# SensorsINI/v2e

Hardware: NVIDIA H100
Metric: Mevents/s (higher is better)
Workload: dtype fp16 tensor-core convs (fp32 accumulate) + f64 pixel state

## Files before the change

### include/v2e_b200.h

```cpp
#ifndef V2E_B200_H
#define V2E_B200_H

#include <stdint.h>

#ifdef __cplusplus
extern "C" {
#endif

typedef enum V2eStatus {
    V2E_OK = 0,
    V2E_E_INVALID = -1,
    V2E_E_CUDA = -2,
    V2E_E_CAPACITY = -3,
    V2E_E_ITER_CAP = -4,
    V2E_E_STATE = -5,
    V2E_E_UNSUPPORTED = -6,
    V2E_E_FALLBACK = -7
} V2eStatus;

typedef enum V2eFrameDtype { V2E_U8 = 0, V2E_F32 = 1, V2E_F64 = 2 } V2eFrameDtype;

const char *v2e_last_error(void);
int v2e_version(void);
int v2e_abi_info(int *version, int *emu_cfg_size, int *frame_info_size, int *unet_weights_size);
// ... 122 lines not shown
    V2E_CONV_TILE_LEGACY = 0,
    V2E_CONV_TILE_256x128 = 1,
    V2E_CONV_TILE_128x256 = 2
};
int v2e_conv2d_lrelu_sm100_tile(const void *x1_dev, int C1, const void *x2_dev, int C2,
                                const void *wgt_dev, const float *bias_dev, int Cout_pad, int KH, int KW,
                                int N, int H, int W, void *out_dev, int out_cstride, int out_mode,
                                int co_real, float slope, int tile, int multicast, void *stream);
int v2e_conv_pick_tile(int C1, int C2, int Cout_pad, int KH, int KW, int N, int H, int W, int n_sms);

int v2e_conv2d_lrelu_sm100_strip(const void *x1_dev, int C1, const void *x2_dev, int C2,
                                 const void *wgt_row_dev, const float *bias_dev, int Cout_pad, int KH,
                                 int KW, int N, int H, int W, void *out_dev, int out_cstride,
                                 int out_mode, int co_real, float slope, void *stream);
int v2e_conv_strip_pick_kc(int C1, int C2, int Cout_pad, int KH, int KW, int W);

int v2e_conv2d_up2_lrelu_sm100(const void *x_low_dev, int C, const void *wgt_fold_dev, const void *wgt_plain_dev,
                               const float *bias_dev, int Cout_pad, int N, int H_out, int W_out, void *out_dev,
                               int out_cstride, float slope, void *stream);
int v2e_conv_up2_fold_weights(const float *w_host, int cout, int cin, int Cout_pad, int C_pad, void *out_host);
int v2e_conv_up2_supported_c(int C, int Cout_pad, int W_out);

typedef struct V2eUNetWeights {
    const float *w[23];
    const float *b[23];
} V2eUNetWeights;

typedef struct V2eSlomo V2eSlomo;

int v2e_slomo_create(int H, int W, int max_batch, const V2eUNetWeights *flow,
// ... 65 lines not shown
```

### v2e_b200/_lib.py

```python
import ctypes
import os

from . import build as _build

_LIB = None


class V2eEmuCfg(ctypes.Structure):
    _fields_ = [
        ("width", ctypes.c_int32), ("height", ctypes.c_int32),
        ("per_pixel_thres", ctypes.c_int32), ("hdr", ctypes.c_int32),
        ("pos_thres_nominal", ctypes.c_double), ("neg_thres_nominal", ctypes.c_double),
        ("cutoff_hz", ctypes.c_double), ("leak_rate_hz", ctypes.c_double),
        ("leak_jitter_fraction", ctypes.c_double), ("refractory_period_s", ctypes.c_double),
        ("shot_noise_rate_hz", ctypes.c_double), ("shot_inten_factor", ctypes.c_double),
        ("rng_mode", ctypes.c_int32), ("iter_cap", ctypes.c_int32),
        ("seed", ctypes.c_uint64),
        ("csdvs", ctypes.c_int32), ("max_frames_per_step", ctypes.c_int32),
        ("cs_tau_p_s", ctypes.c_double), ("cs_tau_h_s", ctypes.c_double),
        ("scidvs", ctypes.c_int32), ("photoreceptor_noise", ctypes.c_int32),
        ("rng_pixel_offset", ctypes.c_uint32), ("full_frame_px", ctypes.c_uint32),
        ("own_row0", ctypes.c_int32), ("own_rows", ctypes.c_int32),
        ("cs_halo_rows", ctypes.c_int32), ("reserved1", ctypes.c_int32),
    ]
# ... 53 lines not shown
    "v2e_emu_cs_max_dev": (_vp, [_vp]),
    "v2e_emu_cs_advance": (_i, [_vp, _i, _i, _vp]),
    "v2e_emu_cs_update": (_i, [_vp, _vp, _i, _vp, _vp, _vp]),
    "v2e_emu_phase_filter": (_i, [_vp, _d, _d, _u64, _i, _vp]),
    "v2e_emu_read_counts": (_i, [_vp, ctypes.POINTER(ctypes.c_int32), _vp, _i, _vp]),
    "v2e_emu_phase_shot": (_i, [_vp, _vp, _i, _d, _d, _vp, _u64, _vp]),
    "v2e_emu_phase_emit": (_i, [_vp, _d, _d, _vp, _u64, _vp]),
    "v2e_conv2d_lrelu_sm100": (_i, [_vp, _i, _vp, _i, _vp, _vp, _i, _i, _i, _i, _i, _i, _vp, _i, _i, _i,
                                    ctypes.c_float, _vp]),
    "v2e_conv2d_lrelu_sm100_tile": (_i, [_vp, _i, _vp, _i, _vp, _vp, _i, _i, _i, _i, _i, _i, _vp, _i, _i, _i,
                                         ctypes.c_float, _i, _i, _vp]),
    "v2e_conv_pick_tile": (_i, [_i, _i, _i, _i, _i, _i, _i, _i, _i]),
    "v2e_conv2d_lrelu_sm100_strip": (_i, [_vp, _i, _vp, _i, _vp, _vp, _i, _i, _i, _i, _i, _i, _vp, _i, _i, _i,
                                          ctypes.c_float, _vp]),
    "v2e_conv_strip_pick_kc": (_i, [_i, _i, _i, _i, _i, _i]),
    "v2e_conv2d_up2_lrelu_sm100": (_i, [_vp, _i, _vp, _vp, _vp, _i, _i, _i, _i, _vp, _i, ctypes.c_float, _vp]),
    "v2e_conv_up2_fold_weights": (_i, [_vp, _i, _i, _i, _i, _vp]),
    "v2e_conv_up2_supported_c": (_i, [_i, _i, _i]),
    "v2e_slomo_create": (_i, [_i, _i, _i, _vp, _vp, ctypes.POINTER(_vp)]),
    "v2e_slomo_destroy": (_i, [_vp]),
    "v2e_slomo_set_pairs": (_i, [_vp, _vp, _i, _vp]),
    "v2e_slomo_max_flow": (_i, [_vp, ctypes.POINTER(ctypes.c_float), _vp]),
    "v2e_slomo_interp": (_i, [_vp, _d, _vp, _vp, _vp]),
    "v2e_slomo_set_option": (_i, [_vp, _i, _i]),
    "v2e_slomo_check_finite": (_i, [_vp, ctypes.POINTER(_i), _vp]),
    "v2e_slomo_profile": (_i, [_vp, _i]),
    "v2e_slomo_profile_read": (_i, [_vp, ctypes.POINTER(ctypes.c_float), ctypes.POINTER(_i),
                                    ctypes.POINTER(ctypes.c_double), _vp]),
    "v2e_slomo_profile_read_layers": (_i, [_vp, ctypes.POINTER(ctypes.c_float), ctypes.POINTER(_i),
                                           ctypes.POINTER(ctypes.c_double), ctypes.POINTER(ctypes.c_float),
# ... 80 lines not shown
```

### v2e_b200/csrc/conv_tc.cu

```cuda
#include <cuda.h>
#include <cuda_fp16.h>
#include <cuda_runtime.h>
#include <math.h>
#include <stdint.h>
#include <stdio.h>
#include <string.h>
#include <vector>
#include <stdlib.h>

#include "../../include/v2e_b200.h"
#include "common.cuh"
#include "tc_common.cuh"

namespace {

constexpr int kTileH = 8, kTileW = 16, kBM = kTileH * kTileW;
constexpr int kStages = 4;
constexpr int kConvThreads = 288;
constexpr int kProducerWarp = 8;
constexpr int kConsumerWarps = 8;

struct ConvParams {
    int N, H, W;
    int C1, C2;
// ... 255 lines not shown

constexpr int kRowTile = 128;

struct StripParams {
    int N, H, W;
    int C1, C2;
    int KH, KW;
    int KC, BN;
    int tiles_x, seg_h, n_seg, n_items;
    int nslot;
    void *pool_out;
    int pool_cstride;
    int n_split, cout_pad;
    int slab_bytes;
    int w_bytes;
    int out_cstride, out_mode, co_real;
    float slope;
    const float *bias;
    void *out;
};
constexpr int kMaxSlot = 12;
constexpr int kStripThreads = 288;

struct RowRing {
    uint64_t *full, *empty;
    uint32_t nslot, cnt;
    int waited, released;
    __device__ __forceinline__ uint32_t slot(int i) const { return (cnt + (uint32_t)i) % nslot; }
    __device__ __forceinline__ void wait_upto(int n) {
        for (; waited < n; waited++) {
            const uint32_t g = cnt + (uint32_t)waited;
            mbar_wait(&full[g % nslot], (g / nslot) & 1u);
        }
    }
    __device__ __forceinline__ void release_upto(int n, int lane) {
        wait_upto(n);
        __syncwarp();
        for (; released < n; released++)
            if (lane == 0) mbar_arrive(&empty[slot(released)]);
    }
};

template <int KW, int KC, int BN>
__device__ __forceinline__ void strip_pair_mma(float (&acc)[2][BN / 2], const RowRing &rr, int row0, int last, int slabs,
                                               uint64_t dr, uint64_t dw, uint32_t a_off, uint32_t row16, uint32_t slab16) {
    constexpr int KH = KW, taps = KH * KW;
    constexpr uint32_t rowb16 = (KC * 2u) >> 4, tile16 = (BN * KC * 2u) >> 4;
#pragma unroll
    for (int k = 0; k < 2; k++) {
#pragma unroll
        for (int i = 0; i < BN / 2; i++) acc[k][i] = 0.f;
        wgmma_fence_regs(acc[k]);
    }
    wgmma_fence();
#pragma unroll
    for (int rp = 0; rp <= KH; rp++) {
        const uint32_t a_row = rr.slot(row0 + (rp < KH ? rp : last)) * row16 + a_off;
        int sl = 0;
#pragma unroll 1
        do {
            const uint32_t a_lo = a_row + (uint32_t)sl * slab16;
#pragma unroll
            for (int s = 0; s < KW; s++) {
#pragma unroll
                for (int j = 0; j < KC / 16; j++) {
                    const uint64_t ad = desc_add(dr, a_lo + (uint32_t)s * rowb16 + 2u * j);
                    if (rp < KH) wgmma_f16<BN>(acc[0], ad, desc_add(dw, (uint32_t)(sl * taps + rp * KW + s) * tile16 + 2u * j), 1u);
                    if (rp > 0) wgmma_f16<BN>(acc[1], ad, desc_add(dw, (uint32_t)(sl * taps + (rp - 1) * KW + s) * tile16 + 2u * j), 1u);
                }
            }
        } while (++sl < slabs);
    }
    wgmma_commit();
}

template <int KW, int KC, int BN, bool POOL>
__global__ void __launch_bounds__(kStripThreads, 1)
conv_strip_kernel(const __grid_constant__ CUtensorMap tmA, const __grid_constant__ CUtensorMap tmA2,
                  const __grid_constant__ CUtensorMap tmB, const StripParams p) {
    extern __shared__ __align__(1024) uint8_t smem_raw[];
    uint8_t *smem = align1024(smem_raw);
    __shared__ __align__(8) uint64_t full_bar[kMaxSlot], empty_bar[kMaxSlot], w_bar;

    constexpr int KH = KW, ph = KH / 2, pw = KW / 2, taps = KH * KW;
    constexpr int PW = kRowTile + KW - 1;
    constexpr uint32_t tile_bytes = BN * KC * 2;
    const int warp = threadIdx.x >> 5, lane = threadIdx.x & 31;
    const int slabs = (p.C1 + p.C2) / KC;
    const uint32_t row_bytes = (uint32_t)p.slab_bytes * slabs;
    uint8_t *ring = smem + ((p.w_bytes + 1023) & ~1023);
    const int split = (int)blockIdx.x % p.n_split, co_off = split * BN;
    const int item0 = (int)blockIdx.x / p.n_split, item_step = (int)gridDim.x / p.n_split;

    if (threadIdx.x == 0) {
        for (int s = 0; s < p.nslot; s++) { mbar_init(&full_bar[s], 1); mbar_init(&empty_bar[s], kConsumerWarps); }
        mbar_init(&w_bar, 1);
        fence_barrier_init();
    }
    if (warp == kProducerWarp && lane == 0) {
        prefetch_tmap(&tmA);
        if (p.C2) prefetch_tmap(&tmA2);
        prefetch_tmap(&tmB);
    }
    __syncthreads();

    if (warp == kProducerWarp) {
        if (lane == 0) {
            mbar_expect_tx(&w_bar, (uint32_t)p.w_bytes);
            for (int t = 0; t < slabs * taps; t++)
                tma_load_2d(smem + (size_t)t * tile_bytes, &tmB, &w_bar, 0, t * p.cout_pad + co_off);
            uint32_t cnt = 0;
            for (int item = item0; item < p.n_items; item += item_step) {
                const int tx = item % p.tiles_x, rest = item / p.tiles_x;
                const int seg = rest % p.n_seg, n = rest / p.n_seg;
                const int ya = seg * p.seg_h, yb = min(p.H, ya + p.seg_h);
                const int x0 = tx * kRowTile;
                for (int i = ya - ph; i < yb + ph; i++, cnt++) {
                    const int slot = (int)(cnt % (uint32_t)p.nslot);
                    mbar_wait(&empty_bar[slot], ((cnt / (uint32_t)p.nslot) & 1u) ^ 1u);
                    mbar_expect_tx(&full_bar[slot], (uint32_t)(PW * KC * 2 * slabs));
                    uint8_t *dst = ring + (size_t)slot * row_bytes;
                    for (int sl = 0; sl < slabs; sl++) {
                        const int c = sl * KC;
                        if (c < p.C1) tma_load_4d(dst + (size_t)sl * p.slab_bytes, &tmA, &full_bar[slot], c, x0 - pw, i, n);
                        else tma_load_4d(dst + (size_t)sl * p.slab_bytes, &tmA2, &full_bar[slot], c - p.C1, x0 - pw, i, n);
// ... 9 lines not shown
        const uint64_t dr = make_smem_desc(smem_u32(ring), swizzle_layout(KC), sbo);
        const uint32_t row16 = row_bytes >> 4, slab16 = (uint32_t)p.slab_bytes >> 4;
        mbar_wait(&w_bar, 0);
        RowRing rr{full_bar, empty_bar, (uint32_t)p.nslot, 0u, 0, 0};
        for (int item = item0; item < p.n_items; item += item_step) {
            const int tx = item % p.tiles_x, rest = item / p.tiles_x;
            const int seg = rest % p.n_seg, n = rest / p.n_seg;
            const int ya = seg * p.seg_h, yb = min(p.H, ya + p.seg_h);
            const int rows_out = yb - ya, rows_in = rows_out + 2 * ph;
            rr.waited = 0; rr.released = 0;
            for (int q = g; 2 * q < rows_out; q += 2) {
                rr.release_upto(2 * q, lane);
                const bool two = 2 * q + 1 < rows_out;
                rr.wait_upto(2 * q + KH + (two ? 1 : 0));
                float acc[2][2][BN / 2];
                auto issue = [&](int hf) {
                    strip_pair_mma<KW, KC, BN>(acc[hf], rr, 2 * q, two ? KH : KH - 1, slabs, dr, dw, hf * half16, row16, slab16);
                };
                const int y = ya + 2 * q;
                auto epilogue = [&](int hf) {
#pragma unroll
                    for (int i = 0; i < 2; i++) {
                        const int m = 64 * hf + 16 * (warp & 3) + (lane >> 2) + 8 * i;
                        const int px = tx * kRowTile + m;
                        const bool inb = px < p.W;
                        const size_t pix = ((size_t)n * p.H + y) * p.W + px;
                        __half2 h0[BN / 8], h1[BN / 8];
                        epilogue_row<BN>(acc[hf][0], i, inb, pix, lane, p.bias + co_off, p.slope, p.out_mode, p.out,
                                         p.out_cstride, co_off, h0);
                        if (two) {
                            epilogue_row<BN>(acc[hf][1], i, inb, pix + p.W, lane, p.bias + co_off, p.slope, p.out_mode, p.out,
                                             p.out_cstride, co_off, h1);
// ... 2 lines not shown
                                    (((size_t)n * (p.H / 2) + y / 2) * (p.W / 2) + px / 2) * p.pool_cstride + co_off);
#pragma unroll
                                for (int j = 0; j < BN / 8; j++) {
                                    const float2 a = __half22float2(h1[j]), b = __half22float2(h0[j]);
                                    float s0 = a.x + b.x, s1 = a.y + b.y;
                                    s0 += __shfl_xor_sync(0xffffffffu, s0, 4);
                                    s1 += __shfl_xor_sync(0xffffffffu, s1, 4);
                                    if (inb && (lane & 4) == 0)
                                        pl[(8 * j + 2 * (lane & 3)) / 2] = __floats2half2_rn(s0 * 0.25f, s1 * 0.25f);
                                }
                            }
                        }
                    }
                };
                if constexpr (kOverlap) {
                    issue(0);
                    issue(1);
                    wgmma_wait<1>();
                    wgmma_fence_regs(acc[0][0]);
                    wgmma_fence_regs(acc[0][1]);
                    epilogue(0);
                    wgmma_wait<0>();
                    wgmma_fence_regs(acc[1][0]);
                    wgmma_fence_regs(acc[1][1]);
                    rr.release_upto(min(rows_in, 2 * q + 4), lane);
                    epilogue(1);
                } else {
#pragma unroll
                    for (int hf = 0; hf < 2; hf++) {
                        issue(hf);
                        wgmma_wait<0>();
                        wgmma_fence_regs(acc[hf][0]);
                        wgmma_fence_regs(acc[hf][1]);
                        if (hf == 1) rr.release_upto(min(rows_in, 2 * q + 4), lane);
                        epilogue(hf);
                    }
                }
            }
            rr.release_upto(rows_in, lane);
            rr.cnt += (uint32_t)rows_in;
        }
    }
}

constexpr int kUpBlocks = 6;
// ... 425 lines not shown
    EncodeTiledFn fn = encode_fn();
    if (!fn) return v2e_set_error(V2E_E_CUDA, "cuTensorMapEncodeTiled unavailable%s", "");
    cuuint64_t dims[4] = {(cuuint64_t)C, (cuuint64_t)W, (cuuint64_t)H, (cuuint64_t)N};
    cuuint64_t strides[3] = {(cuuint64_t)C * 2, (cuuint64_t)W * C * 2, (cuuint64_t)H * W * C * 2};
    cuuint32_t box[4] = {(cuuint32_t)KC, (cuuint32_t)(kRowTile + KW - 1), 1, 1};
    cuuint32_t es[4] = {1, 1, 1, 1};
    CUresult r = fn(tm, CU_TENSOR_MAP_DATA_TYPE_FLOAT16, 4, (void *)ptr, dims, strides, box, es,
                    CU_TENSOR_MAP_INTERLEAVE_NONE, swizzle_for(KC), CU_TENSOR_MAP_L2_PROMOTION_L2_256B,
                    CU_TENSOR_MAP_FLOAT_OOB_FILL_NONE);
    if (r != CUDA_SUCCESS) return v2e_set_error(V2E_E_CUDA, "cuTensorMapEncodeTiled failed for a strip row map%s", "");
    return V2E_OK;
}

constexpr size_t kSmemFull = 222 * 1024, kSmemHalf = 110 * 1024;

static int strip_config(int C1, int C2, int Cout_pad, int KH, int KW, int kc, int *nslot, int *ctas_per_sm, int *n_split) {
    if (Cout_pad > 64) return 0;
    const int slabs = (C1 + C2) / kc;
    const size_t row = (((size_t)(kRowTile + KW - 1) * kc * 2 + 1023) & ~(size_t)1023) * slabs;
    for (int split = 1; split <= 2; split++) {
        const int bn = Cout_pad / split;
        if (bn < 16 || bn % 16) break;
        const size_t wb = ((size_t)slabs * KH * KW * bn * kc * 2 + 1023) & ~(size_t)1023;
        const int two = wb + 2048 + (size_t)(KH + 3) * row <= kSmemHalf;
        const size_t budget = two ? kSmemHalf : kSmemFull;
        if (wb + 2048 + (size_t)(KH + 1) * row > budget) continue;
        int ns = (int)((budget - wb - 2048) / row);
        if (ns > kMaxSlot) ns = kMaxSlot;
        *nslot = ns; *ctas_per_sm = two ? 2 : 1; *n_split = split;
        return 1;
    }
    return 0;
}

static int strip_min_w() {
    static int v = -1;
    if (v < 0) {
        const char *e = getenv("V2E_STRIP_MIN_W");
        v = e ? atoi(e) : 2 * kRowTile;
        if (v < kRowTile) v = kRowTile;
    }
    return v;
}

int v2e_strip_pick(int C1, int C2, int Cout_pad, int KH, int KW, int W, int *nslot_out) {
    if (Cout_pad > 64 || KH != KW || W < strip_min_w() || (KW != 3 && KW != 5 && KW != 7)) return 0;
    const int g = C2 ? (C1 < C2 ? C1 : C2) : C1;
    const int kc = g % 64 == 0 ? 64 : (g % 32 == 0 ? 32 : 16);
    int ns, cps, nsp;
    if (!strip_config(C1, C2, Cout_pad, KH, KW, kc, &ns, &cps, &nsp)) return 0;
    if (nslot_out) *nslot_out = ns;
    return kc;
}

size_t v2e_strip_launch_size(void) { return sizeof(V2eStripLaunch); }

int v2e_strip_pool_supported(int C1, int C2, int Cout_pad, int KH, int KW, int H, int W) {
    if ((H & 1) || (W & 1) || Cout_pad < 32) return 0;
    const int KC = v2e_strip_pick(C1, C2, Cout_pad, KH, KW, W, nullptr);
    if (!((KW == 7 && KC == 32) || (KW == 5 && KC == 64))) return 0;
    int ns, cps, nsp;
    if (!strip_config(C1, C2, Cout_pad, KH, KW, KC, &ns, &cps, &nsp)) return 0;
    return cps == 1 && Cout_pad / nsp >= 32;
}

int v2e_strip_prepare(V2eStripLaunch *L, const void *x1, int C1, const void *x2, int C2, const void *wgt_row,
                      const float *bias, int Cout_pad, int KH, int KW, int N, int H, int W, void *out,
                      int out_cstride, int out_mode, int co_real, float slope, int n_sms, void *pool_out,
                      int pool_cstride) {
    memset(L, 0, sizeof(*L));
    StripParams &p = L->p;
    const int KC = v2e_strip_pick(C1, C2, Cout_pad, KH, KW, W, nullptr);
    int nslot = 0, ctas_per_sm = 0, n_split = 0;
    if (!KC || !strip_config(C1, C2, Cout_pad, KH, KW, KC, &nslot, &ctas_per_sm, &n_split))
        return v2e_set_error(V2E_E_INVALID, "layer does not qualify for the strip kernel%s", "");
    p.N = N; p.H = H; p.W = W; p.C1 = C1; p.C2 = C2; p.KH = KH; p.KW = KW; p.KC = KC;
    p.n_split = n_split; p.cout_pad = Cout_pad; p.BN = Cout_pad / n_split;
    p.tiles_x = (W + kRowTile - 1) / kRowTile;
    int seg_h = H;
    const int strips = p.tiles_x * N;
    while (seg_h > 4 * KH && (long)strips * ((H + seg_h - 1) / seg_h) < 6L * n_sms) seg_h = (seg_h + 1) / 2;
    if (pool_out) {
        if (out_mode != 0 || !v2e_strip_pool_supported(C1, C2, Cout_pad, KH, KW, H, W))
            return v2e_set_error(V2E_E_UNSUPPORTED, "strip: this layer has no pooled epilogue%s", "");
        seg_h = (seg_h + 1) & ~1;
    }
    p.pool_out = pool_out;
    p.pool_cstride = pool_cstride;
    p.seg_h = seg_h;
    p.n_seg = (H + seg_h - 1) / seg_h;
    p.n_items = strips * p.n_seg;
    p.nslot = nslot;
    const int slabs = (C1 + C2) / KC, taps = KH * KW;
    p.slab_bytes = (int)(((size_t)(kRowTile + KW - 1) * KC * 2 + 1023) & ~(size_t)1023);
    p.w_bytes = slabs * taps * p.BN * KC * 2;
    p.out_cstride = out_cstride; p.out_mode = out_mode; p.co_real = co_real; p.slope = slope;
    p.bias = bias; p.out = out;
    int rc;
    if ((rc = make_rowseg_tmap(&L->tmA, x1, N, H, W, C1, KC, KW))) return rc;
    if (C2) { if ((rc = make_rowseg_tmap(&L->tmA2, x2, N, H, W, C2, KC, KW))) return rc; }
    else L->tmA2 = L->tmA;
    {
        EncodeTiledFn fn = encode_fn();
        const int rows_total = slabs * taps * Cout_pad;
        cuuint64_t dims[2] = {(cuuint64_t)KC, (cuuint64_t)rows_total};
        cuuint64_t strides[1] = {(cuuint64_t)KC * 2};
        cuuint32_t box[2] = {(cuuint32_t)KC, (cuuint32_t)p.BN};
        cuuint32_t es[2] = {1, 1};
        CUresult r = fn(&L->tmB, CU_TENSOR_MAP_DATA_TYPE_FLOAT16, 2, (void *)wgt_row, dims, strides, box, es,
                        CU_TENSOR_MAP_INTERLEAVE_NONE, swizzle_for(KC), CU_TENSOR_MAP_L2_PROMOTION_L2_256B,
                        CU_TENSOR_MAP_FLOAT_OOB_FILL_NONE);
        if (r != CUDA_SUCCESS) return v2e_set_error(V2E_E_CUDA, "cuTensorMapEncodeTiled failed for strip weights%s", "");
    }
    L->smem = (size_t)((p.w_bytes + 1023) & ~1023) + (size_t)p.nslot * p.slab_bytes * slabs + 1024;
    int per = ctas_per_sm * n_sms / p.n_split;
    if (per > p.n_items) per = p.n_items;
    if (per < 1) per = 1;
    L->grid = per * p.n_split;
    return V2E_OK;
}

template <int KW, int KC, int BN, bool POOL>
static cudaError_t strip_launch_t(const V2eStripLaunch *L, cudaStream_t st) {
    static PerDeviceOnce attr_once;
    if (attr_once.first())
        cudaFuncSetAttribute(conv_strip_kernel<KW, KC, BN, POOL>, cudaFuncAttributeMaxDynamicSharedMemorySize, 226 * 1024);
    conv_strip_kernel<KW, KC, BN, POOL><<<L->grid, kStripThreads, L->smem, st>>>(L->tmA, L->tmA2, L->tmB, L->p);
    return cudaGetLastError();
}

template <int KW, int KC>
static int strip_launch_kc(const V2eStripLaunch *L, cudaStream_t st, cudaError_t *e) {
    const StripParams &p = L->p;
    if (p.KW != KW || p.KC != KC) return 0;
    if (p.pool_out) {
        if constexpr ((KW == 7 && KC == 32) || (KW == 5 && KC == 64)) {
            if (p.BN == 32) { *e = strip_launch_t<KW, KC, 32, true>(L, st); return 1; }
            if (p.BN == 64) { *e = strip_launch_t<KW, KC, 64, true>(L, st); return 1; }
        }
        return 0;
    }
    if (p.BN == 16) { *e = strip_launch_t<KW, KC, 16, false>(L, st); return 1; }
    if (p.BN == 32) { *e = strip_launch_t<KW, KC, 32, false>(L, st); return 1; }
    if (p.BN == 64) { *e = strip_launch_t<KW, KC, 64, false>(L, st); return 1; }
    return 0;
}

int v2e_strip_launch(const V2eStripLaunch *L, cudaStream_t st) {
    cudaError_t e = cudaSuccess;
    const int launched = strip_launch_kc<3, 16>(L, st, &e) || strip_launch_kc<3, 32>(L, st, &e) ||
                         strip_launch_kc<3, 64>(L, st, &e) || strip_launch_kc<5, 16>(L, st, &e) ||
                         strip_launch_kc<5, 32>(L, st, &e) || strip_launch_kc<5, 64>(L, st, &e) ||
                         strip_launch_kc<7, 16>(L, st, &e) || strip_launch_kc<7, 32>(L, st, &e) ||
                         strip_launch_kc<7, 64>(L, st, &e);
    if (!launched) return v2e_set_error(V2E_E_UNSUPPORTED, "strip kernel: unsupported filter width / slab / pooled epilogue%s", "");
    if (e != cudaSuccess) return v2e_set_error(V2E_E_CUDA, "conv_strip_kernel launch: %s", cudaGetErrorString(e));
    return V2E_OK;
}

extern "C" int v2e_conv2d_lrelu_sm100_strip(const void *x1_dev, int C1, const void *x2_dev, int C2,
                                            const void *wgt_row_dev, const float *bias_dev, int Cout_pad, int KH,
                                            int KW, int N, int H, int W, void *out_dev, int out_cstride,
                                            int out_mode, int co_real, float slope, void *stream) {
    V2eStripLaunch L;
    int dev = 0, sms = 132;
    cudaGetDevice(&dev);
    cudaDeviceGetAttribute(&sms, cudaDevAttrMultiProcessorCount, dev);
    int rc = v2e_strip_prepare(&L, x1_dev, C1, x2_dev, C2, wgt_row_dev, bias_dev, Cout_pad, KH, KW, N, H, W,
                               out_dev, out_cstride, out_mode, co_real, slope, sms, nullptr, 0);
    if (rc) return rc;
    return v2e_strip_launch(&L, (cudaStream_t)stream);
}


struct V2eUpLaunch {
    CUtensorMap tmA, tmB;
    StripParams p;
    int grid;
    size_t smem;
    const __half *low;
    const __half *w_plain;
    int C;
};

int v2e_conv_up2_supported(int C, int Cout_pad, int W_out) {
    if (C != 64 || Cout_pad != 32 || W_out % 2 || W_out < 2 * strip_min_w()) return 0;
// ... 132 lines not shown
```

### v2e_b200/csrc/slomo.cu

```cuda
#include <cuda.h>
#include <cuda_fp16.h>
#include <cuda_runtime.h>
#include <math.h>
#include <stdint.h>
#include <stdio.h>
#include <string.h>
#include <stdlib.h>

#include <vector>

#include "../../include/v2e_b200.h"
#include "common.cuh"

struct V2eConvLaunch;
int v2e_conv_prepare(V2eConvLaunch *L, const void *x1, int C1, const void *x2, int C2, const void *wgt,
                     const float *bias, int Cout_pad, int KH, int KW, int N, int H, int W, void *out,
                     int out_cstride, int out_mode, int co_real, float slope, int tile, int multicast, int n_sms);
int v2e_conv_launch(const V2eConvLaunch *L, cudaStream_t st);
size_t v2e_conv_launch_size(void);
struct V2eStripLaunch;
int v2e_strip_pick(int C1, int C2, int Cout_pad, int KH, int KW, int W, int *nslot_out);
size_t v2e_strip_launch_size(void);
int v2e_strip_pool_supported(int C1, int C2, int Cout_pad, int KH, int KW, int H, int W);
int v2e_strip_prepare(V2eStripLaunch *L, const void *x1, int C1, const void *x2, int C2, const void *wgt_row,
                      const float *bias, int Cout_pad, int KH, int KW, int N, int H, int W, void *out,
                      int out_cstride, int out_mode, int co_real, float slope, int n_sms, void *pool_out,
                      int pool_cstride);
int v2e_strip_launch(const V2eStripLaunch *L, cudaStream_t st);
struct V2eUpLaunch;
int v2e_conv_up2_supported(int C, int Cout_pad, int W_out);
extern "C" int v2e_conv_up2_fold_weights(const float *w, int cout, int cin, int Cout_pad, int C_pad, void *out_host);
size_t v2e_conv_up2_launch_size(void);
int v2e_conv_up2_prepare(V2eUpLaunch *L, const void *x_low, int C, const void *wgt_fold, const void *wgt_plain,
                         const float *bias, int Cout_pad, int N, int H, int W, void *out, int out_cstride, float slope,
                         int n_sms);
int v2e_conv_up2_launch(const V2eUpLaunch *L, cudaStream_t st);
int v2e_set_error(int code, const char *fmt, const char *detail);

#define CU(call)                                                                              \
    do {                                                                                      \
        cudaError_t e_ = (call);                                                              \
        if (e_ != cudaSuccess) return v2e_set_error(V2E_E_CUDA, #call ": %s", cudaGetErrorString(e_)); \
// ... 276 lines not shown

struct V2eSlomo {
    int H, W, maxB;
    UNet flow, interp;
    __half *in16;
    __half *x0, *s1;
    __half *pool[5], *da[5], *s[5];
    __half *up[5], *ua[5], *ub[5];
    float *flow_out, *intrp_out;
    float *img;
    float *maxspeed;
    int *nonfinite;
    int curB;
    std::vector<char> launch_mem, row_mem, up_mem;
    int n_sms, force_tap_kernel, no_fused_up, no_fused_pool;
    int dev_sms;
    int8_t ran[2][23];
    int profile;
    std::vector<cudaEvent_t> ev;
    size_t ev_used;
    double conv_flops;
    std::vector<int> ev_layer;
    std::vector<double> ev_flops;
};

static int layer_level(int i) {
    if (i < 2 || i == 22) return 0;
    if (i < 12) return (i - 2) / 2 + 1;
    return 4 - (i - 12) / 2;
}
// ... 77 lines not shown
        CU(alloc16(&h->ub[k], B * hw * uo[k]));
    }
    CU(cudaMalloc((void **)&h->flow_out, B * HW * 8 * sizeof(float)));
    CU(cudaMalloc((void **)&h->intrp_out, B * HW * 8 * sizeof(float)));
    CU(cudaMalloc((void **)&h->img, (B + 1) * HW * sizeof(float)));
    CU(cudaMalloc((void **)&h->maxspeed, sizeof(float)));
    CU(cudaMalloc((void **)&h->nonfinite, sizeof(int)));
    CU(cudaMemset(h->nonfinite, 0, sizeof(int)));
    h->launch_mem.resize(v2e_conv_launch_size());
    h->row_mem.resize(v2e_strip_launch_size());
    { int dev = 0; cudaGetDevice(&dev); h->n_sms = 132; cudaDeviceGetAttribute(&h->n_sms, cudaDevAttrMultiProcessorCount, dev); }
    h->dev_sms = h->n_sms;
    h->force_tap_kernel = 0;
    h->no_fused_up = getenv("V2E_NO_FUSED_UP") ? 1 : 0;
    h->no_fused_pool = getenv("V2E_NO_FUSED_POOL") ? 1 : 0;
    h->up_mem.resize(v2e_conv_up2_launch_size());
    memset(h->ran, V2E_SLOMO_KERNEL_NONE, sizeof(h->ran));
    *out = h;
    return V2E_OK;
}

extern "C" int v2e_slomo_destroy(V2eSlomo *h) {
    if (!h) return V2E_OK;
    for (UNet *u : {&h->flow, &h->interp})
        for (int i = 0; i < 23; i++) { if (u->w[i]) cudaFree(u->w[i]); if (u->b[i]) cudaFree(u->b[i]); if (u->w_row[i]) cudaFree(u->w_row[i]); if (u->w_fold[i]) cudaFree(u->w_fold[i]); }
    void *ptrs[] = {h->in16, h->x0, h->s1, h->flow_out, h->intrp_out, h->img, h->maxspeed, h->nonfinite};
    for (void *p : ptrs) if (p) cudaFree(p);
    for (int l = 0; l < 5; l++) {
        cudaFree(h->pool[l]); cudaFree(h->da[l]); cudaFree(h->s[l]);
        cudaFree(h->up[l]); cudaFree(h->ua[l]); cudaFree(h->ub[l]);
// ... 2 lines not shown
    delete h;
    return V2E_OK;
}

static int conv(V2eSlomo *h, const UNet &u, int li, const __half *x1, const __half *x2, int B, int H, int W, void *out,
                int out_mode, cudaStream_t st, __half *pool_out = nullptr) {
    int rc;
    const bool row = u.row_kc[li] != 0 && !h->force_tap_kernel;
    V2eConvLaunch *L = (V2eConvLaunch *)h->launch_mem.data();
    V2eStripLaunch *R = (V2eStripLaunch *)h->row_mem.data();
    h->ran[&u == &h->interp][li] = row ? (pool_out ? V2E_SLOMO_KERNEL_STRIP_POOL : V2E_SLOMO_KERNEL_STRIP)
                                       : V2E_SLOMO_KERNEL_TAP;
    if (row)
        rc = v2e_strip_prepare(R, x1, u.c1p[li], x2, x2 ? u.c2p[li] : 0, u.w_row[li], u.b[li], u.cout_pad[li], u.L[li].k,
                               u.L[li].k, B, H, W, out, u.cout_pad[li], out_mode, u.L[li].cout, kSlope, h->n_sms,
                               pool_out, u.cout_pad[li]);
    else
        rc = v2e_conv_prepare(L, x1, u.c1p[li], x2, x2 ? u.c2p[li] : 0, u.w[li], u.b[li], u.cout_pad[li], u.L[li].k,
                              u.L[li].k, B, H, W, out, u.cout_pad[li], out_mode, u.L[li].cout, kSlope,
                              V2E_CONV_TILE_AUTO, 0, h->n_sms);
    if (rc) return rc;
    if (h->profile) {
        if (h->ev_used + 2 > h->ev.size()) {
            size_t old = h->ev.size();
            h->ev.resize(old + 512);
            for (size_t i = old; i < h->ev.size(); i++) cudaEventCreate(&h->ev[i]);
        }
        cudaEventRecord(h->ev[h->ev_used], st);
    }
    rc = row ? v2e_strip_launch(R, st) : v2e_conv_launch(L, st);
    if (h->profile) {
// ... 128 lines not shown
    CU(cudaMemsetAsync(h->nonfinite, 0, sizeof(int), st));
    CU(cudaStreamSynchronize(st));
    return V2E_OK;
}

extern "C" int v2e_slomo_set_option(V2eSlomo *h, int option, int value) {
    if (!h) return v2e_set_error(V2E_E_INVALID, "null handle%s", "");
    if (option == 0) { h->force_tap_kernel = value; return V2E_OK; }
    if (option == 1) { h->no_fused_up = value; return V2E_OK; }
    if (option == 2) { h->no_fused_pool = value; return V2E_OK; }
    if (option == 3) {
        if (value < 0 || value > h->dev_sms) return v2e_set_error(V2E_E_INVALID, "SM count out of range%s", "");
        h->n_sms = value ? value : h->dev_sms;
        return V2E_OK;
    }
    return v2e_set_error(V2E_E_INVALID, "unknown option%s", "");
}

extern "C" int v2e_slomo_profile(V2eSlomo *h, int enable) {
    if (!h) return v2e_set_error(V2E_E_INVALID, "null handle%s", "");
    h->profile = enable ? 1 : 0;
    h->ev_used = 0;
    h->conv_flops = 0;
    h->ev_layer.clear();
    h->ev_flops.clear();
    return V2E_OK;
}

static int profile_collect(V2eSlomo *h, float *conv_ms, int *conv_launches, double *conv_flops, float *ms23, int *n23,
                           double *flops23, void *stream) {
// ... 132 lines not shown
```

### v2e_b200/csrc/tc_common.cuh

```cuda
#pragma once
#include <cuda.h>
#include <cuda_runtime.h>
#include <stdint.h>

__device__ __forceinline__ uint32_t smem_u32(const void *p) { return (uint32_t)__cvta_generic_to_shared(p); }

__device__ __forceinline__ void mbar_init(uint64_t *bar, uint32_t count) {
    asm volatile("mbarrier.init.shared::cta.b64 [%0], %1;" ::"r"(smem_u32(bar)), "r"(count) : "memory");
}
__device__ __forceinline__ void fence_barrier_init() { asm volatile("fence.mbarrier_init.release.cluster;" ::: "memory"); }
__device__ __forceinline__ void mbar_expect_tx(uint64_t *bar, uint32_t bytes) {
    asm volatile("mbarrier.arrive.expect_tx.shared::cta.b64 _, [%0], %1;" ::"r"(smem_u32(bar)), "r"(bytes) : "memory");
}
__device__ __forceinline__ void mbar_arrive(uint64_t *bar) {
    asm volatile("mbarrier.arrive.shared::cta.b64 _, [%0];" ::"r"(smem_u32(bar)) : "memory");
}
__device__ __forceinline__ void mbar_wait(uint64_t *bar, uint32_t parity) {
    const uint32_t addr = smem_u32(bar);
    uint32_t done;
    do {
        asm volatile(
            "{\n\t.reg .pred p;\n\t"
            "mbarrier.try_wait.parity.shared::cta.b64 p, [%1], %2;\n\t"
            "selp.u32 %0, 1, 0, p;\n\t}"
// ... 32 lines not shown
__device__ __forceinline__ void tma_load_2d_multicast(void *dst, const CUtensorMap *tm, uint64_t *bar, int c0, int c1,
                                                      uint16_t mask) {
    asm volatile(
        "cp.async.bulk.tensor.2d.shared::cluster.global.tile.mbarrier::complete_tx::bytes.multicast::cluster"
        " [%0], [%1, {%3, %4}], [%2], %5;"
        ::"r"(smem_u32(dst)), "l"((uint64_t)tm), "r"(smem_u32(bar)), "r"(c0), "r"(c1), "h"(mask) : "memory");
}

__device__ __forceinline__ uint32_t elect_one() {
    uint32_t pred;
    asm volatile("{\n\t.reg .pred p;\n\telect.sync _|p, 0xffffffff;\n\tselp.u32 %0, 1, 0, p;\n\t}" : "=r"(pred));
    return pred;
}

__device__ __forceinline__ void wgmma_fence() { asm volatile("wgmma.fence.sync.aligned;" ::: "memory"); }
__device__ __forceinline__ void wgmma_commit() { asm volatile("wgmma.commit_group.sync.aligned;" ::: "memory"); }
template <int N>
__device__ __forceinline__ void wgmma_wait() { asm volatile("wgmma.wait_group.sync.aligned %0;" ::"n"(N) : "memory"); }
template <int R>
__device__ __forceinline__ void wgmma_fence_regs(float (&d)[R]) {
#pragma unroll
    for (int i = 0; i < R; i++) asm volatile("" : "+f"(d[i])::"memory");
}

__device__ __forceinline__ void wgmma_m64n16k16(float (&d)[8], uint64_t adesc, uint64_t bdesc, uint32_t scale_d) {
    asm volatile(
        "{\n\t.reg .pred p;\n\tsetp.ne.b32 p, %10, 0;\n\t"
        "wgmma.mma_async.sync.aligned.m64n16k16.f32.f16.f16 {%0, %1, %2, %3, %4, %5, %6, %7}, %8, %9, p, 1, 1, 0, 0;\n\t}"
        : "+f"(d[0]), "+f"(d[1]), "+f"(d[2]), "+f"(d[3]), "+f"(d[4]), "+f"(d[5]), "+f"(d[6]), "+f"(d[7])
        : "l"(adesc), "l"(bdesc), "r"(scale_d) : "memory");
// ... 49 lines not shown
```

Baseline: 54.33.

## Stack strip-conv weights so each row pair uses one wider wgmma

Reorders the strip-conv weight tiles in shared memory into a stacked layout, with zero padding, so that the two output rows of a pair share one wgmma of width 2*BN instead of two separate BN-wide wgmmas per input row. The MMA issue is also split into a first group covering the first two input rows and a rest group, so the ring slots for those rows can be released earlier. The cost is extra weight shared memory, which can reduce the number of row-ring slots, plus redundant MMA work on the zero tiles. The stacked path is on by default through an environment variable and a slomo option, and applies only when BN is at most 32.

Result: faster. 55.90, median of 6 (+2.9%).

```diff
diff --git a/include/v2e_b200.h b/include/v2e_b200.h
--- a/include/v2e_b200.h
+++ b/include/v2e_b200.h
@@ -160,6 +160,12 @@
                                  int KW, int N, int H, int W, void *out_dev, int out_cstride,
                                  int out_mode, int co_real, float slope, void *stream);
 int v2e_conv_strip_pick_kc(int C1, int C2, int Cout_pad, int KH, int KW, int W);
+int v2e_conv2d_lrelu_sm100_strip_ex(const void *x1_dev, int C1, const void *x2_dev, int C2,
+                                    const void *wgt_row_dev, const float *bias_dev, int Cout_pad, int KH,
+                                    int KW, int N, int H, int W, void *out_dev, int out_cstride,
+                                    int out_mode, int co_real, float slope, void *pool_out_dev, int pool_cstride,
+                                    int n_sms, int stack, void *stream);
+int v2e_conv_strip_plan(int C1, int C2, int Cout_pad, int KH, int KW, int W, int stack, int *plan4);
 
 int v2e_conv2d_up2_lrelu_sm100(const void *x_low_dev, int C, const void *wgt_fold_dev, const void *wgt_plain_dev,
                                const float *bias_dev, int Cout_pad, int N, int H_out, int W_out, void *out_dev,
diff --git a/v2e_b200/_lib.py b/v2e_b200/_lib.py
--- a/v2e_b200/_lib.py
+++ b/v2e_b200/_lib.py
@@ -91,6 +91,9 @@
     "v2e_conv2d_lrelu_sm100_strip": (_i, [_vp, _i, _vp, _i, _vp, _vp, _i, _i, _i, _i, _i, _i, _vp, _i, _i, _i,
                                           ctypes.c_float, _vp]),
     "v2e_conv_strip_pick_kc": (_i, [_i, _i, _i, _i, _i, _i]),
+    "v2e_conv2d_lrelu_sm100_strip_ex": (_i, [_vp, _i, _vp, _i, _vp, _vp, _i, _i, _i, _i, _i, _i, _vp, _i, _i, _i,
+                                             ctypes.c_float, _vp, _i, _i, _i, _vp]),
+    "v2e_conv_strip_plan": (_i, [_i, _i, _i, _i, _i, _i, _i, ctypes.POINTER(_i)]),
     "v2e_conv2d_up2_lrelu_sm100": (_i, [_vp, _i, _vp, _vp, _vp, _i, _i, _i, _i, _vp, _i, ctypes.c_float, _vp]),
     "v2e_conv_up2_fold_weights": (_i, [_vp, _i, _i, _i, _i, _vp]),
     "v2e_conv_up2_supported_c": (_i, [_i, _i, _i]),
diff --git a/v2e_b200/csrc/conv_tc.cu b/v2e_b200/csrc/conv_tc.cu
--- a/v2e_b200/csrc/conv_tc.cu
+++ b/v2e_b200/csrc/conv_tc.cu
@@ -293,6 +293,7 @@
     int n_split, cout_pad;
     int slab_bytes;
     int w_bytes;
+    int stack;
     int out_cstride, out_mode, co_real;
     float slope;
     const float *bias;
@@ -320,20 +321,25 @@
     }
 };
 
-template <int KW, int KC, int BN>
+__host__ __device__ constexpr int strip_stack_tiles(int KH, int KW) { return KW * (KH + 1) + 1; }
+
+template <int KW, int KC, int BN, bool STACK, int RP0, int RP1>
 __device__ __forceinline__ void strip_pair_mma(float (&acc)[2][BN / 2], const RowRing &rr, int row0, int last, int slabs,
                                                uint64_t dr, uint64_t dw, uint32_t a_off, uint32_t row16, uint32_t slab16) {
-    constexpr int KH = KW, taps = KH * KW;
+    constexpr int KH = KW, taps = KH * KW, stk = strip_stack_tiles(KH, KW);
     constexpr uint32_t rowb16 = (KC * 2u) >> 4, tile16 = (BN * KC * 2u) >> 4;
-#pragma unroll
-    for (int k = 0; k < 2; k++) {
-#pragma unroll
-        for (int i = 0; i < BN / 2; i++) acc[k][i] = 0.f;
-        wgmma_fence_regs(acc[k]);
-    }
-    wgmma_fence();
-#pragma unroll
-    for (int rp = 0; rp <= KH; rp++) {
+    if constexpr (RP0 == 0) {
+#pragma unroll
+        for (int k = 0; k < 2; k++) {
+#pragma unroll
+            for (int i = 0; i < BN / 2; i++) acc[k][i] = 0.f;
+            wgmma_fence_regs(acc[k]);
+        }
+    }
+    float (&both)[BN] = *reinterpret_cast<float (*)[BN]>(&acc[0][0]);
+    if constexpr (RP0 == 0) wgmma_fence();
+#pragma unroll
+    for (int rp = RP0; rp < RP1; rp++) {
         const uint32_t a_row = rr.slot(row0 + (rp < KH ? rp : last)) * row16 + a_off;
         int sl = 0;
 #pragma unroll 1
@@ -344,8 +350,12 @@
 #pragma unroll
                 for (int j = 0; j < KC / 16; j++) {
                     const uint64_t ad = desc_add(dr, a_lo + (uint32_t)s * rowb16 + 2u * j);
-                    if (rp < KH) wgmma_f16<BN>(acc[0], ad, desc_add(dw, (uint32_t)(sl * taps + rp * KW + s) * tile16 + 2u * j), 1u);
-                    if (rp > 0) wgmma_f16<BN>(acc[1], ad, desc_add(dw, (uint32_t)(sl * taps + (rp - 1) * KW + s) * tile16 + 2u * j), 1u);
+                    if constexpr (STACK) {
+                        wgmma_f16<2 * BN>(both, ad, desc_add(dw, (uint32_t)(sl * stk + s * (KH + 1) + KH - rp) * tile16 + 2u * j), 1u);
+                    } else {
+                        if (rp < KH) wgmma_f16<BN>(acc[0], ad, desc_add(dw, (uint32_t)(sl * taps + rp * KW + s) * tile16 + 2u * j), 1u);
+                        if (rp > 0) wgmma_f16<BN>(acc[1], ad, desc_add(dw, (uint32_t)(sl * taps + (rp - 1) * KW + s) * tile16 + 2u * j), 1u);
+                    }
                 }
             }
         } while (++sl < slabs);
@@ -353,7 +363,7 @@
     wgmma_commit();
 }
 
-template <int KW, int KC, int BN, bool POOL>
+template <int KW, int KC, int BN, bool POOL, bool STACK>
 __global__ void __launch_bounds__(kStripThreads, 1)
 conv_strip_kernel(const __grid_constant__ CUtensorMap tmA, const __grid_constant__ CUtensorMap tmA2,
                   const __grid_constant__ CUtensorMap tmB, const StripParams p) {
@@ -361,7 +371,7 @@
     uint8_t *smem = align1024(smem_raw);
     __shared__ __align__(8) uint64_t full_bar[kMaxSlot], empty_bar[kMaxSlot], w_bar;
 
-    constexpr int KH = KW, ph = KH / 2, pw = KW / 2, taps = KH * KW;
+    constexpr int KH = KW, ph = KH / 2, pw = KW / 2, taps = KH * KW, stk = strip_stack_tiles(KH, KW);
     constexpr int PW = kRowTile + KW - 1;
     constexpr uint32_t tile_bytes = BN * KC * 2;
     const int warp = threadIdx.x >> 5, lane = threadIdx.x & 31;
@@ -381,13 +391,24 @@
         if (p.C2) prefetch_tmap(&tmA2);
         prefetch_tmap(&tmB);
     }
+    if constexpr (STACK) {
+        constexpr int per_tile = (int)(tile_bytes / 16);
+        for (int i = threadIdx.x; i < slabs * (KW + 1) * per_tile; i += kStripThreads) {
+            const int z = i / per_tile, sl = z / (KW + 1), s = z % (KW + 1);
+            ((uint4 *)(smem + (size_t)(sl * stk + s * (KH + 1)) * tile_bytes))[i % per_tile] = make_uint4(0u, 0u, 0u, 0u);
+        }
+        fence_proxy_async_shared();
+    }
     __syncthreads();
 
     if (warp == kProducerWarp) {
         if (lane == 0) {
-            mbar_expect_tx(&w_bar, (uint32_t)p.w_bytes);
-            for (int t = 0; t < slabs * taps; t++)
-                tma_load_2d(smem + (size_t)t * tile_bytes, &tmB, &w_bar, 0, t * p.cout_pad + co_off);
+            mbar_expect_tx(&w_bar, (uint32_t)(slabs * taps) * tile_bytes);
+            for (int t = 0; t < slabs * taps; t++) {
+                const int sl = t / taps, r = (t % taps) / KW, s = t % KW;
+                const int dst = STACK ? sl * stk + s * (KH + 1) + (KH - r) : t;
+                tma_load_2d(smem + (size_t)dst * tile_bytes, &tmB, &w_bar, 0, t * p.cout_pad + co_off);
+            }
             uint32_t cnt = 0;
             for (int item = item0; item < p.n_items; item += item_step) {
                 const int tx = item % p.tiles_x, rest = item / p.tiles_x;
@@ -427,8 +448,13 @@
                 const bool two = 2 * q + 1 < rows_out;
                 rr.wait_upto(2 * q + KH + (two ? 1 : 0));
                 float acc[2][2][BN / 2];
-                auto issue = [&](int hf) {
-                    strip_pair_mma<KW, KC, BN>(acc[hf], rr, 2 * q, two ? KH : KH - 1, slabs, dr, dw, hf * half16, row16, slab16);
+                auto issue_first = [&](int hf) {
+                    strip_pair_mma<KW, KC, BN, STACK, 0, 2>(acc[hf], rr, 2 * q, two ? KH : KH - 1, slabs, dr, dw,
+                                                            hf * half16, row16, slab16);
+                };
+                auto issue_rest = [&](int hf) {
+                    strip_pair_mma<KW, KC, BN, STACK, 2, KH + 1>(acc[hf], rr, 2 * q, two ? KH : KH - 1, slabs, dr, dw,
+                                                                 hf * half16, row16, slab16);
                 };
                 const int y = ya + 2 * q;
                 auto epilogue = [&](int hf) {
@@ -461,8 +487,12 @@
                     }
                 };
                 if constexpr (kOverlap) {
-                    issue(0);
-                    issue(1);
+                    issue_first(0);
+                    issue_first(1);
+                    issue_rest(0);
+                    issue_rest(1);
+                    wgmma_wait<2>();
+                    rr.release_upto(2 * q + 2, lane);
                     wgmma_wait<1>();
                     wgmma_fence_regs(acc[0][0]);
                     wgmma_fence_regs(acc[0][1]);
@@ -475,7 +505,12 @@
                 } else {
 #pragma unroll
                     for (int hf = 0; hf < 2; hf++) {
-                        issue(hf);
+                        issue_first(hf);
+                        issue_rest(hf);
+                        if (hf == 1) {
+                            wgmma_wait<1>();
+                            rr.release_upto(2 * q + 2, lane);
+                        }
                         wgmma_wait<0>();
                         wgmma_fence_regs(acc[hf][0]);
                         wgmma_fence_regs(acc[hf][1]);
@@ -931,7 +966,8 @@
 
 constexpr size_t kSmemFull = 222 * 1024, kSmemHalf = 110 * 1024;
 
-static int strip_config(int C1, int C2, int Cout_pad, int KH, int KW, int kc, int *nslot, int *ctas_per_sm, int *n_split) {
+static int strip_config(int C1, int C2, int Cout_pad, int KH, int KW, int kc, int want_stack, int *nslot,
+                        int *ctas_per_sm, int *n_split, int *stack) {
     if (Cout_pad > 64) return 0;
     const int slabs = (C1 + C2) / kc;
     const size_t row = (((size_t)(kRowTile + KW - 1) * kc * 2 + 1023) & ~(size_t)1023) * slabs;
@@ -944,10 +980,22 @@
         if (wb + 2048 + (size_t)(KH + 1) * row > budget) continue;
         int ns = (int)((budget - wb - 2048) / row);
         if (ns > kMaxSlot) ns = kMaxSlot;
-        *nslot = ns; *ctas_per_sm = two ? 2 : 1; *n_split = split;
+        *nslot = ns; *ctas_per_sm = two ? 2 : 1; *n_split = split; *stack = 0;
+        const size_t wbs = ((size_t)slabs * strip_stack_tiles(KH, KW) * bn * kc * 2 + 1023) & ~(size_t)1023;
+        if (want_stack && bn <= 32 && wbs + 2048 <= budget) {
+            int nss = (int)((budget - wbs - 2048) / row);
+            if (nss > kMaxSlot) nss = kMaxSlot;
+            if (nss >= (ns < KH + 3 ? ns : KH + 3)) { *nslot = nss; *stack = 1; }
+        }
         return 1;
     }
     return 0;
+}
+
+static int strip_stack_env() {
+    static int v = -1;
+    if (v < 0) { const char *e = getenv("V2E_STRIP_STACK"); v = e ? (atoi(e) != 0) : 1; }
+    return v;
 }
 
 static int strip_min_w() {
@@ -964,8 +1012,8 @@
     if (Cout_pad > 64 || KH != KW || W < strip_min_w() || (KW != 3 && KW != 5 && KW != 7)) return 0;
     const int g = C2 ? (C1 < C2 ? C1 : C2) : C1;
     const int kc = g % 64 == 0 ? 64 : (g % 32 == 0 ? 32 : 16);
-    int ns, cps, nsp;
-    if (!strip_config(C1, C2, Cout_pad, KH, KW, kc, &ns, &cps, &nsp)) return 0;
+    int ns, cps, nsp, stk;
+    if (!strip_config(C1, C2, Cout_pad, KH, KW, kc, 0, &ns, &cps, &nsp, &stk)) return 0;
     if (nslot_out) *nslot_out = ns;
     return kc;
 }
@@ -976,20 +1024,20 @@
     if ((H & 1) || (W & 1) || Cout_pad < 32) return 0;
     const int KC = v2e_strip_pick(C1, C2, Cout_pad, KH, KW, W, nullptr);
     if (!((KW == 7 && KC == 32) || (KW == 5 && KC == 64))) return 0;
-    int ns, cps, nsp;
-    if (!strip_config(C1, C2, Cout_pad, KH, KW, KC, &ns, &cps, &nsp)) return 0;
+    int ns, cps, nsp, stk;
+    if (!strip_config(C1, C2, Cout_pad, KH, KW, KC, 0, &ns, &cps, &nsp, &stk)) return 0;
     return cps == 1 && Cout_pad / nsp >= 32;
 }
 
 int v2e_strip_prepare(V2eStripLaunch *L, const void *x1, int C1, const void *x2, int C2, const void *wgt_row,
                       const float *bias, int Cout_pad, int KH, int KW, int N, int H, int W, void *out,
                       int out_cstride, int out_mode, int co_real, float slope, int n_sms, void *pool_out,
-                      int pool_cstride) {
+                      int pool_cstride, int stack) {
     memset(L, 0, sizeof(*L));
     StripParams &p = L->p;
     const int KC = v2e_strip_pick(C1, C2, Cout_pad, KH, KW, W, nullptr);
     int nslot = 0, ctas_per_sm = 0, n_split = 0;
-    if (!KC || !strip_config(C1, C2, Cout_pad, KH, KW, KC, &nslot, &ctas_per_sm, &n_split))
+    if (!KC || !strip_config(C1, C2, Cout_pad, KH, KW, KC, stack, &nslot, &ctas_per_sm, &n_split, &p.stack))
         return v2e_set_error(V2E_E_INVALID, "layer does not qualify for the strip kernel%s", "");
     p.N = N; p.H = H; p.W = W; p.C1 = C1; p.C2 = C2; p.KH = KH; p.KW = KW; p.KC = KC;
     p.n_split = n_split; p.cout_pad = Cout_pad; p.BN = Cout_pad / n_split;
@@ -1010,7 +1058,7 @@
     p.nslot = nslot;
     const int slabs = (C1 + C2) / KC, taps = KH * KW;
     p.slab_bytes = (int)(((size_t)(kRowTile + KW - 1) * KC * 2 + 1023) & ~(size_t)1023);
-    p.w_bytes = slabs * taps * p.BN * KC * 2;
+    p.w_bytes = slabs * (p.stack ? strip_stack_tiles(KH, KW) : taps) * p.BN * KC * 2;
     p.out_cstride = out_cstride; p.out_mode = out_mode; p.co_real = co_real; p.slope = slope;
     p.bias = bias; p.out = out;
     int rc;
@@ -1037,12 +1085,12 @@
     return V2E_OK;
 }
 
-template <int KW, int KC, int BN, bool POOL>
+template <int KW, int KC, int BN, bool POOL, bool STACK = false>
 static cudaError_t strip_launch_t(const V2eStripLaunch *L, cudaStream_t st) {
     static PerDeviceOnce attr_once;
     if (attr_once.first())
-        cudaFuncSetAttribute(conv_strip_kernel<KW, KC, BN, POOL>, cudaFuncAttributeMaxDynamicSharedMemorySize, 226 * 1024);
-    conv_strip_kernel<KW, KC, BN, POOL><<<L->grid, kStripThreads, L->smem, st>>>(L->tmA, L->tmA2, L->tmB, L->p);
+        cudaFuncSetAttribute(conv_strip_kernel<KW, KC, BN, POOL, STACK>, cudaFuncAttributeMaxDynamicSharedMemorySize, 226 * 1024);
+    conv_strip_kernel<KW, KC, BN, POOL, STACK><<<L->grid, kStripThreads, L->smem, st>>>(L->tmA, L->tmA2, L->tmB, L->p);
     return cudaGetLastError();
 }
 
@@ -1052,9 +1100,20 @@
     if (p.KW != KW || p.KC != KC) return 0;
     if (p.pool_out) {
         if constexpr ((KW == 7 && KC == 32) || (KW == 5 && KC == 64)) {
+            if (p.stack) {
+                if constexpr (KW == 7) {
+                    if (p.BN == 32) { *e = strip_launch_t<KW, KC, 32, true, true>(L, st); return 1; }
+                }
+                return 0;
+            }
             if (p.BN == 32) { *e = strip_launch_t<KW, KC, 32, true>(L, st); return 1; }
             if (p.BN == 64) { *e = strip_launch_t<KW, KC, 64, true>(L, st); return 1; }
         }
+        return 0;
+    }
+    if (p.stack) {
+        if (p.BN == 16) { *e = strip_launch_t<KW, KC, 16, false, true>(L, st); return 1; }
+        if (p.BN == 32) { *e = strip_launch_t<KW, KC, 32, false, true>(L, st); return 1; }
         return 0;
     }
     if (p.BN == 16) { *e = strip_launch_t<KW, KC, 16, false>(L, st); return 1; }
@@ -1084,9 +1143,34 @@
     cudaGetDevice(&dev);
     cudaDeviceGetAttribute(&sms, cudaDevAttrMultiProcessorCount, dev);
     int rc = v2e_strip_prepare(&L, x1_dev, C1, x2_dev, C2, wgt_row_dev, bias_dev, Cout_pad, KH, KW, N, H, W,
-                               out_dev, out_cstride, out_mode, co_real, slope, sms, nullptr, 0);
+                               out_dev, out_cstride, out_mode, co_real, slope, sms, nullptr, 0, strip_stack_env());
     if (rc) return rc;
     return v2e_strip_launch(&L, (cudaStream_t)stream);
+}
+
+extern "C" int v2e_conv2d_lrelu_sm100_strip_ex(const void *x1_dev, int C1, const void *x2_dev, int C2,
+                                               const void *wgt_row_dev, const float *bias_dev, int Cout_pad, int KH,
+                                               int KW, int N, int H, int W, void *out_dev, int out_cstride,
+                                               int out_mode, int co_real, float slope, void *pool_out_dev,
+                                               int pool_cstride, int n_sms, int stack, void *stream) {
+    if (stack < -1 || stack > 1) return v2e_set_error(V2E_E_INVALID, "stack must be -1, 0 or 1%s", "");
+    const int sms = device_sms();
+    if (n_sms < 0 || n_sms > sms) return v2e_set_error(V2E_E_INVALID, "SM count out of range%s", "");
+    V2eStripLaunch L;
+    int rc = v2e_strip_prepare(&L, x1_dev, C1, x2_dev, C2, wgt_row_dev, bias_dev, Cout_pad, KH, KW, N, H, W,
+                               out_dev, out_cstride, out_mode, co_real, slope, n_sms ? n_sms : sms, pool_out_dev,
+                               pool_cstride, stack < 0 ? strip_stack_env() : stack);
+    if (rc) return rc;
+    return v2e_strip_launch(&L, (cudaStream_t)stream);
+}
+
+extern "C" int v2e_conv_strip_plan(int C1, int C2, int Cout_pad, int KH, int KW, int W, int stack, int *plan4) {
+    if (!plan4) return v2e_set_error(V2E_E_INVALID, "null argument%s", "");
+    const int kc = v2e_strip_pick(C1, C2, Cout_pad, KH, KW, W, nullptr);
+    plan4[0] = plan4[1] = plan4[2] = plan4[3] = 0;
+    if (kc) strip_config(C1, C2, Cout_pad, KH, KW, kc, stack < 0 ? strip_stack_env() : stack, &plan4[2], &plan4[1],
+                         &plan4[3], &plan4[0]);
+    return kc;
 }
 
 
diff --git a/v2e_b200/csrc/slomo.cu b/v2e_b200/csrc/slomo.cu
--- a/v2e_b200/csrc/slomo.cu
+++ b/v2e_b200/csrc/slomo.cu
@@ -25,7 +25,7 @@
 int v2e_strip_prepare(V2eStripLaunch *L, const void *x1, int C1, const void *x2, int C2, const void *wgt_row,
                       const float *bias, int Cout_pad, int KH, int KW, int N, int H, int W, void *out,
                       int out_cstride, int out_mode, int co_real, float slope, int n_sms, void *pool_out,
-                      int pool_cstride);
+                      int pool_cstride, int stack);
 int v2e_strip_launch(const V2eStripLaunch *L, cudaStream_t st);
 struct V2eUpLaunch;
 int v2e_conv_up2_supported(int C, int Cout_pad, int W_out);
@@ -332,6 +332,7 @@
     int curB;
     std::vector<char> launch_mem, row_mem, up_mem;
     int n_sms, force_tap_kernel, no_fused_up, no_fused_pool;
+    int strip_stack;
     int dev_sms;
     int8_t ran[2][23];
     int profile;
@@ -439,6 +440,7 @@
     h->force_tap_kernel = 0;
     h->no_fused_up = getenv("V2E_NO_FUSED_UP") ? 1 : 0;
     h->no_fused_pool = getenv("V2E_NO_FUSED_POOL") ? 1 : 0;
+    { const char *e = getenv("V2E_STRIP_STACK"); h->strip_stack = e ? (atoi(e) != 0) : 1; }
     h->up_mem.resize(v2e_conv_up2_launch_size());
     memset(h->ran, V2E_SLOMO_KERNEL_NONE, sizeof(h->ran));
     *out = h;
@@ -471,7 +473,7 @@
     if (row)
         rc = v2e_strip_prepare(R, x1, u.c1p[li], x2, x2 ? u.c2p[li] : 0, u.w_row[li], u.b[li], u.cout_pad[li], u.L[li].k,
                                u.L[li].k, B, H, W, out, u.cout_pad[li], out_mode, u.L[li].cout, kSlope, h->n_sms,
-                               pool_out, u.cout_pad[li]);
+                               pool_out, u.cout_pad[li], h->strip_stack);
     else
         rc = v2e_conv_prepare(L, x1, u.c1p[li], x2, x2 ? u.c2p[li] : 0, u.w[li], u.b[li], u.cout_pad[li], u.L[li].k,
                               u.L[li].k, B, H, W, out, u.cout_pad[li], out_mode, u.L[li].cout, kSlope,
@@ -630,6 +632,7 @@
         h->n_sms = value ? value : h->dev_sms;
         return V2E_OK;
     }
+    if (option == 4) { h->strip_stack = value != 0; return V2E_OK; }
     return v2e_set_error(V2E_E_INVALID, "unknown option%s", "");
 }
 
diff --git a/v2e_b200/csrc/tc_common.cuh b/v2e_b200/csrc/tc_common.cuh
--- a/v2e_b200/csrc/tc_common.cuh
+++ b/v2e_b200/csrc/tc_common.cuh
@@ -70,6 +70,7 @@
 }
 
 __device__ __forceinline__ void wgmma_fence() { asm volatile("wgmma.fence.sync.aligned;" ::: "memory"); }
+__device__ __forceinline__ void fence_proxy_async_shared() { asm volatile("fence.proxy.async.shared::cta;" ::: "memory"); }
 __device__ __forceinline__ void wgmma_commit() { asm volatile("wgmma.commit_group.sync.aligned;" ::: "memory"); }
 template <int N>
 __device__ __forceinline__ void wgmma_wait() { asm volatile("wgmma.wait_group.sync.aligned %0;" ::"n"(N) : "memory"); }
```
